# SCLBD/Accelerated-Lpbox-ADMM

Hardware: AMD Instinct MI355X
Metric: admm_iters_per_sec_batched_lp_j100_k500 (higher is better)
Workload: dtype f64

## Files before the change

accelerated-lpbox-admm_amd/csrc/lpbox_dev_common.h:

```cpp
#pragma once
#include <hip/hip_runtime.h>

namespace {

template <int CTRL>
__device__ __forceinline__ double dpp_mov(double v) {
    int lo = __double2loint(v), hi = __double2hiint(v);
    lo = __builtin_amdgcn_mov_dpp(lo, CTRL, 0xf, 0xf, true);
    hi = __builtin_amdgcn_mov_dpp(hi, CTRL, 0xf, 0xf, true);
    return __hiloint2double(hi, lo);
}

struct HalfSwap {
    static __device__ __forceinline__ void run(double a, double b, double &r0, double &r1) {
        auto lo = __builtin_amdgcn_permlane32_swap(__double2loint(a), __double2loint(b), false, false);
        auto hi = __builtin_amdgcn_permlane32_swap(__double2hiint(a), __double2hiint(b), false, false);
        r0 = __hiloint2double(hi[0], lo[0]); r1 = __hiloint2double(hi[1], lo[1]);
    }
};
struct RowSwap {
    static __device__ __forceinline__ void run(double a, double b, double &r0, double &r1) {
        auto lo = __builtin_amdgcn_permlane16_swap(__double2loint(a), __double2loint(b), false, false);
        auto hi = __builtin_amdgcn_permlane16_swap(__double2hiint(a), __double2hiint(b), false, false);
        r0 = __hiloint2double(hi[0], lo[0]); r1 = __hiloint2double(hi[1], lo[1]);
    }
};
template <typename SWAP>
__device__ __forceinline__ double pair_step(double a, double b) { double r0, r1; SWAP::run(a, b, r0, r1); return r0 + r1; }

__device__ __forceinline__ double row_allreduce(double v) {
    v = v + dpp_mov<0xB1>(v);
    v = v + dpp_mov<0x4E>(v);
    v = v + dpp_mov<0x141>(v);
    v = v + dpp_mov<0x140>(v);
    return v;
}

__device__ __forceinline__ double wave_allreduce_sum(double v) {
#ifdef LPBOX_REDUCE_SHFL
    v = v + __shfl_xor(v, 32, 64); v = v + __shfl_xor(v, 16, 64);
    for (int off = 1; off < 16; off <<= 1) v = v + __shfl_xor(v, off, 64);
    return v;
#else
    v = pair_step<HalfSwap>(v, v);
    v = pair_step<RowSwap>(v, v);
    return row_allreduce(v);
#endif
}

template <int NV>
__device__ __forceinline__ double wave_reduce_scatter(const double *v) {
    static_assert(NV >= 2 && NV <= 4, "2..4 values");
    const double x = pair_step<HalfSwap>(v[0], v[1]);
    double s;
    if constexpr (NV == 2) s = pair_step<RowSwap>(x, x);
    else {
        const double y = NV == 4 ? pair_step<HalfSwap>(v[2], v[3]) : pair_step<HalfSwap>(v[2], v[2]);
        s = pair_step<RowSwap>(x, y);
    }
    return row_allreduce(s);
}
__device__ __forceinline__ constexpr int scatter_lane(int nv, int k) { return nv == 2 ? 32 * k : (k == 0 ? 0 : k == 1 ? 32 : k == 2 ? 16 : 48); }

__device__ __forceinline__ int wave_max_int(int v) {
    for (int off = 1; off < 64; off <<= 1) { int o = __shfl_xor(v, off, 64); v = o > v ? o : v; }
    return __builtin_amdgcn_readfirstlane(v);
}

constexpr int RED_MAXV = 6;
constexpr int RED_MAXW = 16;

constexpr int RED_STAGE_BCAST = 0;
constexpr int RED_STAGE_PAIRS = 1;

template <int NV>
__device__ __forceinline__ void wave_partials_store(const double *v, double *buf, int lane, int w) {
    const int row = lane >> 4, k = ((row & 1) << 1) | (row >> 1);
    const bool owner = (lane & 15) == 0;
    double *at = buf + k * RED_MAXW + w;
    if constexpr (NV == 1) {
        const double t0 = wave_allreduce_sum(v[0]);
        if (owner) *at = t0;
    } else {
        constexpr int NS4 = NV > 4 ? 4 : NV;
        const double sc = wave_reduce_scatter<NS4>(v);
        if constexpr (NV == 6) {
            const double sc2 = wave_reduce_scatter<2>(v + 4);
            if (owner) { *at = sc; buf[(4 + (k & 1)) * RED_MAXW + w] = sc2; }
        } else {
            static_assert(NV <= 4, "1, 2, 3, 4 or 6 values");
            if (owner) *at = sc;
        }
    }
}

template <int T, int NV, int STAGE = RED_STAGE_BCAST>
__device__ __forceinline__ void block_sum(double (&v)[NV], double *red, int &parity) {
    constexpr int W = T / 64;
    static_assert(W == 1 || W == 2 || W == 4 || W == 8 || W == 16, "waves per workgroup");
    if constexpr (W == 1) {
#pragma unroll
        for (int k = 0; k < NV; k++) v[k] = wave_allreduce_sum(v[k]);
        return;
    }
    const int lane = threadIdx.x & 63, w = threadIdx.x >> 6;
    double *buf = red + parity * (RED_MAXV * RED_MAXW);
    if constexpr (STAGE != RED_STAGE_BCAST) {
        static_assert(W == 8 && STAGE == RED_STAGE_PAIRS, "built for eight waves");
        wave_partials_store<NV>(v, buf, lane, w);
        __syncthreads();
        double2 t[NV];
#pragma unroll
        for (int k = 0; k < NV; k++) t[k] = *(const double2 *)(buf + k * RED_MAXW + 2 * (lane & 3));
#pragma unroll
        for (int k = 0; k < NV; k++) {
            double u = t[k].x + t[k].y;
            u = u + dpp_mov<0xB1>(u);
            u = u + dpp_mov<0x4E>(u);
            v[k] = u;
        }
        parity ^= 1;
        return;
    }
    if constexpr (NV == 1) {
        const double t0 = wave_allreduce_sum(v[0]);
        if (lane == 0) buf[w] = t0;
    } else {
        constexpr int NS4 = NV > 4 ? 4 : NV;
        const double sc = wave_reduce_scatter<NS4>(v);
#pragma unroll
        for (int k = 0; k < NS4; k++) if (lane == scatter_lane(NS4, k)) buf[k * RED_MAXW + w] = sc;
        if constexpr (NV == 5) {
            const double t4 = wave_allreduce_sum(v[4]);
            if (lane == 0) buf[4 * RED_MAXW + w] = t4;
        } else if constexpr (NV == 6) {
            const double sc2 = wave_reduce_scatter<2>(v + 4);
#pragma unroll
            for (int k = 0; k < 2; k++) if (lane == scatter_lane(2, k)) buf[(4 + k) * RED_MAXW + w] = sc2;
        } else static_assert(NV <= 4, "at most six values");
    }
    __syncthreads();
    if constexpr (W >= 16) {
        double t[NV];
#pragma unroll
        for (int k = 0; k < NV; k++) t[k] = buf[k * RED_MAXW + (lane & (W - 1))];
#pragma unroll
        for (int k = 0; k < NV; k++) v[k] = row_allreduce(t[k]);
        parity ^= 1;
        return;
    }
    double t[NV][W];
#pragma unroll
    for (int k = 0; k < NV; k++)
#pragma unroll
        for (int w2 = 0; w2 < W; w2++) t[k][w2] = buf[k * RED_MAXW + w2];
#pragma unroll
    for (int k = 0; k < NV; k++) {
#pragma unroll
        for (int span = 1; span < W; span <<= 1)
#pragma unroll
            for (int w2 = 0; w2 < W; w2 += 2 * span) t[k][w2] = t[k][w2] + t[k][w2 + span];
        v[k] = t[k][0];
// ... 46 lines not shown
```

accelerated-lpbox-admm_amd/csrc/lpbox_lp_kernels.hip:

```cpp
#include "lpbox_lp.h"
#include "lpbox_dev_common.h"

#include <float.h>

#include <utility>

namespace {

#ifdef LPBOX_STAMPS
#define STAMP_DECL unsigned long long st_acc[16] = {0}; unsigned long long st_t = __builtin_amdgcn_s_memtime();
#define STAMP(k) { __builtin_amdgcn_sched_barrier(0); unsigned long long st_n = __builtin_amdgcn_s_memtime(); \
                   __builtin_amdgcn_s_waitcnt(0xC07F); st_acc[k] += st_n - st_t; st_t = st_n; __builtin_amdgcn_sched_barrier(0); }
#define STAMP_STORE if (tid == 64 * bd.stamp_wave && bd.stamps) { for (int k = 0; k < 16; k++) bd.stamps[(size_t)inst * 16 + k] = st_acc[k]; }
#else
#define STAMP_DECL
#define STAMP(k)
#define STAMP_STORE
#endif
#if defined(LPBOX_STAMPS) && defined(LPBOX_STAMPS_PREBAR)
#define STAMP_PRE(k) STAMP(k)
#define STAMP_POST(k) STAMP(14)
#else
#define STAMP_PRE(k)
#define STAMP_POST(k) STAMP(k)
#endif

#ifndef LPBOX_LP_G1
#define LPBOX_LP_G1 2
#endif
#if !defined(LPBOX_STAMPS) && !defined(LPBOX_KO_COLCAP) && !defined(LPBOX_KO_ROWCAP) && !defined(LPBOX_KO_NOMUL) && !defined(LPBOX_KO_ROWS) && \
    !defined(LPBOX_KO_COLS) && !defined(LPBOX_KO_RED1) && !defined(LPBOX_KO_RED2) && !defined(LPBOX_KO_DIV) && !defined(LPBOX_KO_FIXED_PCG) && LPBOX_LP_G1 == 2
#define LPBOX_PCG_SPEC 1
#else
#define LPBOX_PCG_SPEC 0
#endif
#if LPBOX_PCG_SPEC && !defined(LPBOX_LP_OUTER_LEGACY)
#define LPBOX_OUTER_FUSED 1
#else
#define LPBOX_OUTER_FUSED 0
#endif

struct LdsLayout {
    size_t gx, gl, red, hist, rowf, rowy3, rs_ptr, cs_ptr, hs_ptr, rs_col, cs_row, H, dcol, drow, dmap, total;
    __host__ __device__ LdsLayout(int NS, int LS, int ZS, bool lean, int HL = 0, int HLD = 0) {
        size_t o = 0;
        auto take = [&](size_t bytes) { size_t at = o; o += (bytes + 15) & ~size_t(15); return at; };
        gx = take(sizeof(double) * (2 * (size_t)NS + 3));
        gl = take(sizeof(double) * 3 * ((size_t)LS + 1));
        red = take(sizeof(double) * 2 * RED_MAXV * RED_MAXW);
        hist = take(sizeof(double) * 2 * LP_HIST);
        rowf = take(lean ? sizeof(double) * ((size_t)LS + 1) : 0);
        rowy3 = take(lean ? sizeof(double) * ((size_t)LS + 1) : 0);
        rs_ptr = take(sizeof(int) * ((size_t)NS + 1));
        cs_ptr = take(sizeof(int) * ((size_t)NS + 1));
        hs_ptr = take(sizeof(int) * ((size_t)NS + 1));
        rs_col = take(sizeof(uint16_t) * (size_t)ZS);
        cs_row = take(sizeof(uint16_t) * (size_t)ZS);
        H = take(sizeof(double) * (size_t)HL * (size_t)HLD);
        dcol = take(HL ? sizeof(double) * ((size_t)HL + 1) : 0);
        drow = take(HL ? sizeof(double) * ((size_t)HL + 1) : 0);
        dmap = take(HL ? sizeof(int) * ((size_t)HL + 1) : 0);
        total = o;
    }
};

__host__ __device__ constexpr bool lp_is_lean(int T, int EPT) { return EPT >= 4 || T == 1024; }

__host__ __device__ constexpr int lp_red_stage(int T, int EPT) {
    return T == 512 && EPT == 1 ? RED_STAGE_PAIRS : RED_STAGE_BCAST;
}

constexpr int LP_PCG_RCAP = 12, LP_PCG_CCAP = 12, LP_PCG_HCAP = 8;
__host__ __device__ constexpr bool lp_pcg_scalar_loop(int T, int EPT, bool direct, bool log) { return LPBOX_PCG_SPEC != 0 && T == 512 && EPT == 1 && !direct && !log; }
__host__ __device__ constexpr bool lp_pcg_spec_geometry(int T, int EPT, bool direct, bool log) { return lp_pcg_scalar_loop(T, EPT, direct, log); }
__host__ __device__ constexpr bool lp_pcg_spec_built(int rn, int cn, int hn) {
    return rn >= 0 && rn <= LP_PCG_RCAP / 2 && cn >= 0 && cn <= LP_PCG_CCAP / 2 && hn >= 0 && hn <= LP_PCG_HCAP / 2;
}
__host__ __device__ constexpr bool lp_outer_fused(int T, int EPT, bool direct, bool log) { return LPBOX_OUTER_FUSED != 0 && T == 512 && EPT == 1 && !direct && !log; }

typedef __attribute__((address_space(3))) double lds_double;

__device__ __forceinline__ unsigned lds_addr(const void *p) {
    return (unsigned)(size_t)(__attribute__((address_space(3))) const void *)p;
}
template <int COMP>
__device__ __forceinline__ double lds_ld(unsigned a) {
    return ((const lds_double *)(size_t)a)[COMP];
}

template <int... V>
struct Caps {
    static constexpr int N = sizeof...(V);
    static constexpr int total = (V + ... + 0);
    static constexpr int at(int i) { constexpr int a[N] = {V...}; return a[i]; }
    static constexpr int off(int i) { constexpr int a[N] = {V...}; int o = 0; for (int k = 0; k < i; k++) o += a[k]; return o; }
};

template <typename F, int... I>
__device__ __forceinline__ void static_for_impl(F &&f, std::integer_sequence<int, I...>) {
    (f(std::integral_constant<int, I>{}), ...);
}
template <int N, typename F>
__device__ __forceinline__ void static_for(F &&f) {
    static_for_impl(f, std::make_integer_sequence<int, N>{});
}

template <typename C>
struct Lists {
    unsigned addr[C::total > 0 ? C::total : 1];
    const int *ptr;
    int pos0, pstride;
    int tail_any[C::N];
    static constexpr bool TAILREG = C::N < 4;
    int tail_begin[TAILREG ? C::N : 1], tail_end[TAILREG ? C::N : 1];
    int wlen[C::N];
    unsigned base, zero;
};

template <typename C, int S, int STRIDE>
__device__ __forceinline__ void build_list(Lists<C> &g, int begin, int end, const uint16_t *idx) {
    constexpr int CAP = C::at(S), OFF = C::off(S);
#pragma unroll
    for (int k = 0; k < CAP; k++) g.addr[OFF + k] = (begin + k < end) ? g.base + STRIDE * (unsigned)idx[begin + k] : g.zero;
// ... 268 lines not shown
    }
    __device__ __forceinline__ void load(double *uniform_base, unsigned thread_idx) {
        ub = (char *)uniform_base; boff = thread_idx * 8u;
        if constexpr (MODE != 1) {
#pragma unroll
            for (int s = 0; s < N; s++) r[s] = *elem(s);
        }
    }
    __device__ __forceinline__ double get(int s) const { if constexpr (MODE == 1) return *elem(s); else return r[s]; }
    __device__ __forceinline__ void set(int s, double v) { if constexpr (MODE == 1) *elem(s) = v; else r[s] = v; }
    __device__ __forceinline__ void park(bool dirty = true) {
        if constexpr (MODE == 2) {
            if (dirty) {
#pragma unroll
                for (int s = 0; s < N; s++) *elem(s) = r[s];
            }
        }
    }
    __device__ __forceinline__ void unpark() {
        if constexpr (MODE == 2) {
#pragma unroll
            for (int s = 0; s < N; s++) r[s] = *elem(s);
        }
    }
    __device__ __forceinline__ void store() const {
        if constexpr (MODE != 1) {
#pragma unroll
            for (int s = 0; s < N; s++) *elem(s) = r[s];
        }
    }
};

template <bool MEM, int N, int STRIDE>
struct RowVec {
    double r[MEM ? 1 : N];
    double *lds;
    static __device__ __forceinline__ int at(int idx) {
#ifndef LPBOX_NO_OPAQUE_ROWVEC
        asm volatile("" : "+v"(idx));
#endif
        return idx * STRIDE;
    }
    __device__ __forceinline__ double get(int s, int idx, bool leader) const {
        if constexpr (MEM) return leader ? lds[at(idx)] : 0.0; else return r[s];
    }
    __device__ __forceinline__ void set(int s, int idx, bool leader, double v) {
        if constexpr (MEM) { if (leader) lds[at(idx)] = v; } else r[s] = v;
    }
};

template <int T, int EPT, typename RCAPS, typename CCAPS, typename HCAPS, bool DIRECT = false, bool LOG = false>
__global__ void __launch_bounds__(T) lp_window_kernel(LpBatchDev bd, int iter_start, int iter_end, int mode) {
    const int l2f = mode & 1, rec = mode & 2;
    constexpr int RS = (DIRECT || LOG) ? RED_STAGE_BCAST : lp_red_stage(T, EPT);
    constexpr bool SCALAR_LOOP = lp_pcg_scalar_loop(T, EPT, DIRECT, LOG), SPEC = lp_pcg_spec_geometry(T, EPT, DIRECT, LOG);
    constexpr bool FUSED = lp_outer_fused(T, EPT, DIRECT, LOG);
    auto uni = [](bool c) { if constexpr (SCALAR_LOOP) return __builtin_amdgcn_ballot_w64(c) != 0; else return c; };
    extern __shared__ __attribute__((aligned(16))) unsigned char smem[];
    const int inst = blockIdx.x, tid = threadIdx.x;
    int *isc = bd.isc + (size_t)inst * NI_COUNT;
    double *dsc = bd.dsc + (size_t)inst * ND_COUNT;
    if (!isc[NI_ACTIVE]) return;

    const int nnz = isc[NI_NNZ];
    const size_t on = (size_t)inst * bd.NS, ol = (size_t)inst * bd.LS, oz = (size_t)inst * bd.ZS;

    static_assert(!DIRECT || EPT == 1, "the direct x-update is built for the one-slot variants");
    const LdsLayout L(bd.NS, bd.LS, bd.ZS, lp_is_lean(T, EPT), DIRECT ? bd.HL : 0, DIRECT ? bd.HLD : 0);
    double *gx = (double *)(smem + L.gx);
    double *gl = (double *)(smem + L.gl);
    double *red = (double *)(smem + L.red);
    double *s_hist = (double *)(smem + L.hist);
    int *s_rs_ptr = (int *)(smem + L.rs_ptr);
    int *s_cs_ptr = (int *)(smem + L.cs_ptr);
    int *s_hs_ptr = (int *)(smem + L.hs_ptr);
    uint16_t *s_rs_col = (uint16_t *)(smem + L.rs_col);
    uint16_t *s_cs_row = (uint16_t *)(smem + L.cs_row);

    {
        const int *gp = bd.rs_ptr + (size_t)inst * (bd.NS + 1);
        const int *gc = bd.cs_ptr + (size_t)inst * (bd.NS + 1);
        const int *gh = bd.hs_ptr + (size_t)inst * (bd.NS + 1);
        for (int i = tid; i <= bd.NS; i += T) { s_rs_ptr[i] = gp[i]; s_cs_ptr[i] = gc[i]; s_hs_ptr[i] = gh[i]; }
        const uint16_t *c0 = bd.rs_col + oz, *r0 = bd.cs_row + oz;
        for (int k = tid; k < nnz; k += T) { s_rs_col[k] = c0[k]; s_cs_row[k] = r0[k]; }
        if (tid == 0) { gx[bd.NS] = 0.0; gx[2 * bd.NS + 2] = 0.0; gl[3 * bd.LS] = 0.0; gl[3 * bd.LS + 1] = 0.0; gl[3 * bd.LS + 2] = 0.0; }
    }
    double *Hm = (double *)(smem + L.H), *dcol = (double *)(smem + L.dcol), *drow = (double *)(smem + L.drow);
    int *dmap = (int *)(smem + L.dmap);
    int h_valid = 0;
    if constexpr (DIRECT) {
        h_valid = isc[NI_H_VALID];
        const size_t hsz = (size_t)bd.HL * bd.HLD;
        if (h_valid) { const double *Hg = bd.H + (size_t)inst * (hsz + bd.LS); for (size_t e = tid; e < hsz; e += T) Hm[e] = Hg[e]; }
    }

    constexpr bool LEAN = lp_is_lean(T, EPT);
    double x[EPT], dinv[EPT];
    SlotVec<LEAN ? 2 : 0, EPT, T> z1, z2, b;
    SlotVec<LEAN ? 1 : 0, EPT, T> pd;
    z1.load(bd.z1 + on, (unsigned)tid); z2.load(bd.z2 + on, (unsigned)tid); b.load(bd.b + on, (unsigned)tid); pd.load(bd.pd + on, (unsigned)tid);
    double Esq_reg[LEAN ? 1 : EPT];
    if constexpr (!LEAN) {
#pragma unroll
        for (int s = 0; s < EPT; s++) Esq_reg[s] = (double)(bd.cmeta[on + s * T + tid] & 0x7FFF);
    }
    auto Esq = [&](int s) { if constexpr (LEAN) return (double)(bd.cmeta[on + s * T + tid] & 0x7FFF); else return Esq_reg[s]; };
    bool live[EPT];
    double Ex[EPT];
    RowVec<LEAN, EPT, 3> z4;
    RowVec<LEAN, EPT, 1> f, y3;
    z4.lds = gl + 1; f.lds = (double *)(smem + L.rowf); y3.lds = (double *)(smem + L.rowy3);
    int rinfo[EPT], rGreg[LEAN ? 1 : EPT];
    bool rvreg[LEAN ? 1 : EPT];
    auto rgl = [&](int s) { return rinfo[s] & 0xFFFF; };
    auto rG = [&](int s) { if constexpr (LEAN) return (rinfo[s] >> 16) & 15; else return rGreg[s]; };
    auto rvalid = [&](int s) { if constexpr (LEAN) return (rinfo[s] & (1 << 20)) != 0; else return rvreg[s]; };
#pragma unroll
    for (int s = 0; s < EPT; s++) {
        const int pos = s * T + tid;
        x[s] = bd.x[on + pos];
        live[s] = bd.live[on + pos] != 0;
        const int rid = bd.rid[on + pos], meta = bd.rmeta[on + pos];
        const bool rtask = rid != 0xFFFF, leader = rtask && (meta & 15) == 0;
        rinfo[s] = rtask ? ((int)bd.rgl[on + pos] | ((meta >> 4) << 16) | (leader ? 1 << 20 : 0)) : (1 << 16);
        if constexpr (!LEAN) { rinfo[s] &= 0xFFFF; rGreg[s] = rtask ? (meta >> 4) : 1; rvreg[s] = leader; }
        z4.set(s, rgl(s), leader, leader ? bd.z4[ol + rid] : 0.0);
        f.set(s, rgl(s), leader, leader ? bd.f[ol + rid] : 0.0);
        y3.set(s, rgl(s), leader, 0.0);
        Ex[s] = 0.0;
    }
    int gdir = -1;
    double wrow = 0.0;
    if constexpr (DIRECT) {
        if (rvalid(0)) {
            gdir = bd.rdir[on + tid];
            if (gdir >= 0) dmap[gdir] = rgl(0);
            if (h_valid) wrow = bd.H[(size_t)inst * ((size_t)bd.HL * bd.HLD + bd.LS) + (size_t)bd.HL * bd.HLD + rgl(0)];
            gl[3 * rgl(0) + 2] = 0.0;
        }
    }
    double rho1 = dsc[ND_RHO1], rho2 = dsc[ND_RHO2], rho4 = dsc[ND_RHO4];
    double prev_rho1 = dsc[ND_PREV_RHO1], prev_rho2 = dsc[ND_PREV_RHO2], prev_rho4 = dsc[ND_PREV_RHO4];
    double gamma_val = dsc[ND_GAMMA], dI = dsc[ND_DI], r4Et = dsc[ND_R4ET], rcr = dsc[ND_RCR];
    double std_obj = dsc[ND_STD_OBJ], cur_obj = dsc[ND_CUR_OBJ], best_bin_obj = dsc[ND_BEST_BIN_OBJ];
    double sum_fix_obj = dsc[ND_SUM_FIX_OBJ], fix_obj = dsc[ND_FIX_OBJ], c1 = dsc[ND_C1];
    double cvg1 = dsc[ND_CVG1], cvg2 = dsc[ND_CVG2], obj_val = dsc[ND_OBJ_VAL];
    double prev_sum = dsc[ND_PREV_SUM], prev_obj = dsc[ND_PREV_OBJ];
    int n_live = isc[NI_NLIVE], rhoUpdated = isc[NI_RHO_UPDATED], hist_n = isc[NI_HIST_N];
    int pcg_total = isc[NI_PCG_TOTAL], outer_total = isc[NI_OUTER_TOTAL], last_pcg = isc[NI_LAST_PCG];
    int expr_ready = isc[NI_EXPR_READY];
    int hbuf = 0;
    double h_reg[LEAN ? 1 : LP_HIST];
    if constexpr (LEAN) { if (tid < LP_HIST) s_hist[tid] = bd.hist[(size_t)inst * LP_HIST + tid]; }
    else {
#pragma unroll
        for (int k = 0; k < LP_HIST; k++) h_reg[k] = bd.hist[(size_t)inst * LP_HIST + k];
    }
    const double learning_fact = LP_LEARNING_FACT;
    int ret = 0, stop = LP_STOP_NONE, parity = 0;

    __syncthreads();

    static_assert(RCAPS::N == EPT && CCAPS::N == EPT && HCAPS::N == EPT, "one capacity per slot");
    Lists<RCAPS> rl;
    Lists<CCAPS> cl;
    Lists<HCAPS> hl;
    bool clong[EPT];
    int anyhelp[EPT];
    rl.base = lds_addr(gx); rl.zero = lds_addr(gx + bd.NS);
    rl.ptr = s_rs_ptr; cl.ptr = s_cs_ptr; hl.ptr = s_hs_ptr;
    rl.pos0 = cl.pos0 = hl.pos0 = tid; rl.pstride = cl.pstride = hl.pstride = T;
    cl.base = lds_addr(gl); cl.zero = lds_addr(gl + 3 * bd.LS);
    hl.base = cl.base; hl.zero = cl.zero;
    int rGmax[EPT];
    static_for<EPT>([&](auto S) {
        constexpr int s = decltype(S)::value;
        const int pos = s * T + tid;
        build_list<RCAPS, s, 8>(rl, s_rs_ptr[pos], s_rs_ptr[pos + 1], s_rs_col);
        rGmax[s] = wave_max_int(rG(s));
        build_list<CCAPS, s, 24>(cl, s_cs_ptr[pos], s_cs_ptr[pos + 1], s_cs_row);
        build_list<HCAPS, s, 24>(hl, s_hs_ptr[pos], s_hs_ptr[pos + 1], s_cs_row);
        const int cm = bd.cmeta[on + pos];
        clong[s] = (cm & 0x8000) != 0;
        anyhelp[s] = wave_max_int(s_hs_ptr[pos + 1] - s_hs_ptr[pos]) > 0;
    });
    int spec_rn = 0, spec_cn = 0, spec_hn = 0;
    bool spec_ok = false;
    if constexpr (SPEC) {
        static_assert(RCAPS::at(0) == LP_PCG_RCAP && CCAPS::at(0) == LP_PCG_CCAP && HCAPS::at(0) == LP_PCG_HCAP, "capacities of the 512 x 1 kernel");
        spec_rn = (rl.wlen[0] + 1) / 2; spec_cn = (cl.wlen[0] + 1) / 2; spec_hn = (hl.wlen[0] + 1) / 2;
        spec_ok = !bd.pcg_generic && !(rl.tail_any[0] | cl.tail_any[0] | hl.tail_any[0]);
    }
    auto op_add = [](double acc, double v) { return acc + v; };
    constexpr int GX2 = T * EPT + 2;
    auto rows_combine = [&](const double (&part)[EPT], double (&out)[EPT]) {
        static_for<EPT>([&](auto S) {
            constexpr int s = decltype(S)::value;
            double v = part[s];
            if (rGmax[s] >= 2) { const double u = v + dpp_mov<0xB1>(v); v = rG(s) >= 2 ? u : v; }
            if (rGmax[s] >= 4) { const double u = v + dpp_mov<0x4E>(v); v = rG(s) >= 4 ? u : v; }
            if (rGmax[s] >= 8) { const double u = v + dpp_mov<0x141>(v); v = rG(s) >= 8 ? u : v; }
            out[s] = v;
        });
    };
    auto rows_gather_at = [&](auto COMPC, double (&out)[EPT]) {
        double part[EPT];
        if constexpr (LEAN) touch_list(rl);
        gather_all<RCAPS, 8, decltype(COMPC)::value>(rl, s_rs_col, op_add, part);
        rows_combine(part, out);
    };
    auto rows_gather = [&](double (&out)[EPT]) { rows_gather_at(std::integral_constant<int, 0>{}, out); };

// ... 290 lines not shown
                            const int j = tid & 127;
                            if (j < nG) {
                                const double rk = drow[j];
                                for (int i = tid >> 7; i < nG; i += T / 128) {
                                    const double ck = dcol[i];
                                    const double cur = Hm[i * HLD + j];
                                    Hm[i * HLD + j] = i == k ? rk : (j == k ? -(ck * piv) : cur - ck * rk);
                                }
                            }
                        }
                        __syncthreads();
                    }
                    {
                        double *Hg = bd.H + (size_t)inst * ((size_t)bd.HL * HLD + bd.LS);
                        for (int e = tid; e < bd.HL * HLD; e += T) Hg[e] = Hm[e];
                        if (rvalid(0)) Hg[(size_t)bd.HL * HLD + rgl(0)] = wrow;
                    }
                    h_valid = 1;
                }
                const double q1 = apply_Q(rhs[0]);
                gx[tid] = live[0] ? q1 : 0.0;
                __syncthreads();
                {
                    double t[EPT];
                    rows_gather(t);
                    if (rvalid(0) && gdir >= 0) dcol[gdir] = t[0];
                }
                __syncthreads();
                for (int i = tid >> 2; i < nG; i += T / 4) {
                    const double *Hr = Hm + i * HLD;
                    double acc = 0.0;
#pragma unroll 4
                    for (int j = tid & 3; j < nG; j += 4) acc = acc + Hr[j] * dcol[j];
                    const double u = quad_sum(acc);
                    if ((tid & 3) == 0) gl[3 * dmap[i] + 2] = u;
                }
                __syncthreads();
                double v[EPT];
                cols_gather(std::integral_constant<int, 2>{}, op_add, v);
                const double yv = rhs[0] - v[0];
                xt[0] = apply_Q(yv) / dI;
            } else {
            double r[EPT], p[EPT];
            double p3[3] = {0.0, 0.0, 0.0};
            double tcol[EPT];
            if constexpr (FUSED) tcol[0] = tcf[0];
            else
            cols_gather(std::integral_constant<int, 2>{}, op_add, tcol);
#pragma unroll
            for (int s = 0; s < EPT; s++) {
                const double t = tcol[s];
                xt[s] = y1[s];
                double Mx = 0.0;
                Mx += dI * (1.0 * xt[s]);
                Mx += t;
                r[s] = rhs[s] - Mx;
                p[s] = dinv[s] * r[s];
                p3[0] = p3[0] + (live[s] ? rhs[s] * rhs[s] : 0.0);
                p3[1] = p3[1] + (live[s] ? r[s] * r[s] : 0.0);
                p3[2] = p3[2] + (live[s] ? r[s] * p[s] : 0.0);
            }
            block_sum<T, 3, RS>(p3, red, parity);
            STAMP(2)
            const double rhsNorm2 = p3[0];
            double residualNorm2 = p3[1], absNew = p3[2];
            if (uni(rhsNorm2 == 0)) {
#pragma unroll
                for (int s = 0; s < EPT; s++) xt[s] = 0.0;
            } else {
                double threshold = LP_PCG_TOL * LP_PCG_TOL * rhsNorm2;
                if (threshold < DBL_MIN) threshold = DBL_MIN;
                if constexpr (SCALAR_LOOP) {
                    auto pcg_loop = [&](auto RKC, auto CKC, auto HKC) {
                        constexpr int RK = decltype(RKC)::value, CK = decltype(CKC)::value, HK = decltype(HKC)::value;
                        static_assert((RK >= 0) == (CK >= 0) && (RK >= 0) == (HK >= 0) && (RK < 0 || EPT == 1), "all three lists or none");
                        while (k_it < LP_PCG_MAXITERS) {
#pragma unroll
                            for (int s = 0; s < EPT; s++) gx[s * T + tid] = live[s] ? p[s] : 0.0;
                            __syncthreads();
                            {
                                double q[EPT];
                                if constexpr (RK >= 0) {
                                    double v[RK > 0 ? RK * LPBOX_LP_G1 : 1], part[EPT];
                                    list_read<0, RK>(rl, v);
                                    part[0] = list_sum<RK>(v, op_add);
                                    rows_combine(part, q);
                                } else rows_gather(q);
#pragma unroll
                                for (int s = 0; s < EPT; s++) if (rvalid(s)) gl[3 * rgl(s)] = r4 * q[s];
                            }
                            __syncthreads();
                            double tmp[EPT];
                            double p1[1] = {0.0};
                            if constexpr (CK >= 0) {
                                double vo[CK > 0 ? CK * LPBOX_LP_G1 : 1], vh[HK > 0 ? HK * LPBOX_LP_G1 : 1];
                                list_read<0, CK>(cl, vo);
                                const double own = list_sum<CK>(vo, op_add);
                                __builtin_amdgcn_sched_barrier(0);
                                list_read<0, HK>(hl, vh);
                                if constexpr (HK > 0) {
                                    const double ht = quad_sum(list_sum<HK>(vh, op_add));
                                    tcol[0] = clong[0] ? own + ht : own;
                                } else tcol[0] = own;
                            } else cols_gather(std::integral_constant<int, 0>{}, op_add, tcol);
#pragma unroll
                            for (int s = 0; s < EPT; s++) {
                                const double t = tcol[s];
                                double Mp = 0.0;
                                Mp += dI * (1.0 * p[s]);
                                Mp += t;
                                tmp[s] = Mp;
                                p1[0] = p1[0] + (live[s] ? p[s] * tmp[s] : 0.0);
                            }
                            block_sum<T, 1, RS>(p1, red, parity);
                            const double alpha = absNew / p1[0];
                            if (uni(alpha < 0)) { pcg_fail = true; break; }
                            double p2[2] = {0.0, 0.0};
                            double z[EPT];
#pragma unroll
                            for (int s = 0; s < EPT; s++) {
                                xt[s] += alpha * p[s];
                                r[s] -= alpha * tmp[s];
                                z[s] = dinv[s] * r[s];
                                p2[0] = p2[0] + (live[s] ? r[s] * r[s] : 0.0);
                                p2[1] = p2[1] + (live[s] ? r[s] * z[s] : 0.0);
                            }
                            block_sum<T, 2, RS>(p2, red, parity);
                            residualNorm2 = p2[0];
                            if (uni(residualNorm2 < threshold)) { k_it++; break; }
                            const double absOld = absNew;
                            absNew = p2[1];
                            const double beta = absNew / absOld;
#pragma unroll
                            for (int s = 0; s < EPT; s++) p[s] = z[s] + beta * p[s];
                            k_it++;
                        }
                    };
                    constexpr std::integral_constant<int, -1> GEN{};
                    if (uni(!(residualNorm2 < threshold))) {
                        if constexpr (SPEC) {
                            bool ran = false;
                            if (spec_ok) {
                                dispatch_chunks<LP_PCG_RCAP / 2>(spec_rn, [&](auto R) {
                                    dispatch_chunks<LP_PCG_CCAP / 2>(spec_cn, [&](auto Cn) {
                                        dispatch_chunks<LP_PCG_HCAP / 2>(spec_hn, [&](auto H) {
                                            if constexpr (lp_pcg_spec_built(decltype(R)::value, decltype(Cn)::value, decltype(H)::value)) {
                                                pcg_loop(R, Cn, H);
                                                ran = true;
                                            }
                                        });
                                    });
                                });
                            }
                            if (!ran) pcg_loop(GEN, GEN, GEN);
                        } else pcg_loop(GEN, GEN, GEN);
                    }
                } else {
                if (!(residualNorm2 < threshold)) {
                    while (k_it < LP_PCG_MAXITERS) {
#pragma unroll
                        for (int s = 0; s < EPT; s++) gx[s * T + tid] = live[s] ? p[s] : 0.0;
                        STAMP_PRE(12)
                        __syncthreads();
                        STAMP(3)
                        {
                            double q[EPT];
#ifdef LPBOX_KO_ROWS
                            for (int s = 0; s < EPT; s++) q[s] = p[s];
#else
                            rows_gather(q);
#endif
                            STAMP(4)
#pragma unroll
#ifdef LPBOX_KO_NOMUL
                            for (int s = 0; s < EPT; s++) if (rvalid(s)) gl[3 * rgl(s)] = q[s];
#else
                            for (int s = 0; s < EPT; s++) if (rvalid(s)) gl[3 * rgl(s)] = r4 * q[s];
#endif
// ... 95 lines not shown
                z1.set(s, z1.get(s) + g1 * (x[s] - y1[s]));
                z2.set(s, z2.get(s) + g2 * (x[s] - y2[s]));
                gx[s * T + tid] = live[s] ? x[s] : 0.0;
            }
            if constexpr (FUSED) {
                const bool step = (it + 1) % LP_RHO_STEP == 0;
                start_vec(step ? learning_fact * rho1 : rho1);
                r4n = step ? learning_fact * r4Et : r4Et;
            }
            __syncthreads();
            if constexpr (FUSED) rows_gather_x_y1(Ex, qn);
            else
            rows_gather(Ex);
#pragma unroll
            for (int s = 0; s < EPT; s++) {
                if constexpr (LEAN) {
                    if (rvalid(s)) {
                        const int i = RowVec<true, EPT, 1>::at(rgl(s));
                        const double d = g4 * ((Ex[s] + y3.lds[i]) - f.lds[i]);
                        const double z4o = z4.lds[3 * i];
                        z4.lds[3 * i] = (!l2f && it == iter_start) ? d : z4o + d;
                    }
                } else {
                const double d = g4 * ((Ex[s] + y3.get(s, rgl(s), rvalid(s))) - f.get(s, rgl(s), rvalid(s)));
                z4.set(s, rgl(s), rvalid(s), (!l2f && it == iter_start) ? d : z4.get(s, rgl(s), rvalid(s)) + d);
                }
            }
            double lg[6] = {0.0, 0.0, 0.0, 0.0, 0.0, 0.0};
            if constexpr (LOG) {
#pragma unroll
                for (int s = 0; s < EPT; s++) {
                    const double vy3 = y3.get(s, rgl(s), rvalid(s)), vz4 = z4.get(s, rgl(s), rvalid(s));
                    lg[0] = lg[0] + (live[s] ? y1[s] * y1[s] : 0.0);
                    lg[1] = lg[1] + (live[s] ? y2[s] * y2[s] : 0.0);
                    lg[2] = lg[2] + (rvalid(s) ? vy3 * vy3 : 0.0);
                    lg[3] = lg[3] + (live[s] ? z1.get(s) * z1.get(s) : 0.0);
                    lg[4] = lg[4] + (live[s] ? z2.get(s) * z2.get(s) : 0.0);
                    lg[5] = lg[5] + (rvalid(s) ? vz4 * vz4 : 0.0);
                }
            }
            const bool rho_step = (it + 1) % LP_RHO_STEP == 0;
            double p5[6] = {0.0, 0.0, 0.0, 0.0, 0.0, 0.0};
            p5[5] = prepare(rho_step ? learning_fact * rho1 : rho1, rho_step ? learning_fact * rho2 : rho2, rho_step ? learning_fact * rho4 : rho4);
#pragma unroll
            for (int s = 0; s < EPT; s++) {
                const double d1 = x[s] - y1[s], d2 = x[s] - y2[s];
                const double xb = x[s] >= 0.5 ? 1.0 : 0.0;
                p5[0] = p5[0] + (live[s] ? x[s] * x[s] : 0.0);
                p5[1] = p5[1] + (live[s] ? d1 * d1 : 0.0);
                p5[2] = p5[2] + (live[s] ? d2 * d2 : 0.0);
                p5[3] = p5[3] + (live[s] ? b.get(s) * x[s] : 0.0);
                p5[4] = p5[4] + (live[s] ? b.get(s) * xb : 0.0);
            }
            STAMP_POST(12)
            block_sum<T, 6, RS>(p5, red, parity);
            if constexpr (LOG) block_sum<T, 6, RS>(lg, red, parity);
            pnorm = p5[5];
            STAMP_POST(13)
            {
                const double xn = sqrt(p5[0]);
                const double temp0 = (xn < 2.2204e-16) ? 2.2204e-16 : xn;
                cvg1 = sqrt(p5[1]) / temp0;
                cvg2 = sqrt(p5[2]) / temp0;
            }
            if (cvg1 <= LP_STOP_THRESHOLD && cvg2 <= LP_STOP_THRESHOLD && (l2f || it != iter_start)) {
                if (l2f) ret = 1;
                stop = LP_STOP_Y1Y2;
                break;
            }
            if (rho_step) {
                prev_rho1 = rho1; prev_rho2 = rho2;
                rho1 = learning_fact * rho1;
                rho2 = learning_fact * rho2;
                prev_rho4 = rho4;
                rho4 = learning_fact * rho4;
                const double g = gamma_val * LP_GAMMA_FACTOR;
                gamma_val = g < 1.0 ? 1.0 : g;
                rhoUpdated = 1;
                rcr = learning_fact - 1.0;
            }
            obj_val = p5[3];
            double h[LP_HIST];
            if constexpr (LEAN) {
                const double *hs = s_hist + hbuf * LP_HIST;
#pragma unroll
                for (int k = 0; k < LP_HIST; k++) h[k] = hs[k];
            } else {
#pragma unroll
                for (int k = 0; k < LP_HIST; k++) h[k] = h_reg[k];
            }
            if (hist_n < LP_HIST) {
#pragma unroll
                for (int k = 0; k < LP_HIST; k++) if (k == hist_n) h[k] = obj_val;
            } else {
#pragma unroll
                for (int k = 0; k < LP_HIST - 1; k++) h[k] = h[k + 1];
                h[LP_HIST - 1] = obj_val;
            }
            if constexpr (LEAN) {
                hbuf ^= 1;
                if (tid == 0) {
#pragma unroll
                    for (int k = 0; k < LP_HIST; k++) s_hist[hbuf * LP_HIST + k] = h[k];
                }
            } else {
#pragma unroll
                for (int k = 0; k < LP_HIST; k++) h_reg[k] = h[k];
            }
            if (hist_n < 0x3fffffff) hist_n++;
            if (hist_n >= LP_HIST) {
                double mean = 0;
#pragma unroll
                for (int k = 0; k < LP_HIST; k++) mean += h[k];
                mean /= (double)LP_HIST;
                double dev = 0;
#pragma unroll
                for (int k = 0; k < LP_HIST; k++) dev += (h[k] - mean) * (h[k] - mean);
                dev /= (double)(LP_HIST - 1);
                const double sd = (dev == 0) ? 0.0 : sqrt(dev);
                std_obj = sd / fabs(h[LP_HIST - 1]);
            }
            if (std_obj <= LP_STD_THRESHOLD) { ret = 1; stop = LP_STOP_OBJSTD; break; }
            cur_obj = p5[4];
            if (best_bin_obj >= cur_obj) best_bin_obj = cur_obj;
            if constexpr (LOG) {
                if (tid == 0 && bd.logbuf && it - iter_start < bd.log_cap) {
                    double *lr = bd.logbuf + ((size_t)inst * bd.log_cap + (it - iter_start)) * LP_LOG_VALS;
                    lr[0] = (double)k_it; lr[1] = sqrt(p5[0]);
#pragma unroll
                    for (int k = 0; k < 6; k++) lr[2 + k] = sqrt(lg[k]);
                    lr[8] = obj_val; lr[9] = cur_obj; lr[10] = (double)(wall_clock64() - log_t0); lr[11] = (double)it;
                }
            }
            if constexpr (LEAN) {
                rho1 = uniform_f64(rho1); rho2 = uniform_f64(rho2); rho4 = uniform_f64(rho4);
                prev_rho1 = uniform_f64(prev_rho1); prev_rho2 = uniform_f64(prev_rho2); prev_rho4 = uniform_f64(prev_rho4);
                gamma_val = uniform_f64(gamma_val); rcr = uniform_f64(rcr); dI = uniform_f64(dI); r4Et = uniform_f64(r4Et);
                std_obj = uniform_f64(std_obj); cur_obj = uniform_f64(cur_obj); best_bin_obj = uniform_f64(best_bin_obj);
                cvg1 = uniform_f64(cvg1); cvg2 = uniform_f64(cvg2); obj_val = uniform_f64(obj_val); pnorm = uniform_f64(pnorm);
            }
            STAMP(14)
        }
        STAMP_STORE
    }

    z1.store(); z2.store(); pd.store();
#pragma unroll
    for (int s = 0; s < EPT; s++) {
        const int pos = s * T + tid;
        {
            bd.x[on + pos] = x[s];
            bd.live[on + pos] = live[s] ? 1 : 0;
        }
        if (rvalid(s)) { const int rid = bd.rid[on + pos]; bd.z4[ol + rid] = z4.get(s, rgl(s), true); bd.f[ol + rid] = f.get(s, rgl(s), true); }
    }
    if (tid == 0) {
        dsc[ND_RHO1] = rho1; dsc[ND_RHO2] = rho2; dsc[ND_RHO4] = rho4;
        dsc[ND_PREV_RHO1] = prev_rho1; dsc[ND_PREV_RHO2] = prev_rho2; dsc[ND_PREV_RHO4] = prev_rho4;
        dsc[ND_GAMMA] = gamma_val; dsc[ND_DI] = dI; dsc[ND_R4ET] = r4Et; dsc[ND_RCR] = rcr;
        dsc[ND_STD_OBJ] = std_obj; dsc[ND_CUR_OBJ] = cur_obj; dsc[ND_BEST_BIN_OBJ] = best_bin_obj;
        dsc[ND_SUM_FIX_OBJ] = sum_fix_obj; dsc[ND_FIX_OBJ] = fix_obj; dsc[ND_C1] = c1;
        dsc[ND_CVG1] = cvg1; dsc[ND_CVG2] = cvg2; dsc[ND_OBJ_VAL] = obj_val;
        dsc[ND_PREV_SUM] = prev_sum; dsc[ND_PREV_OBJ] = prev_obj;
        isc[NI_NLIVE] = n_live; isc[NI_RHO_UPDATED] = rhoUpdated; isc[NI_HIST_N] = hist_n;
        isc[NI_RET] = ret; isc[NI_STOP] = stop;
        isc[NI_PCG_TOTAL] = pcg_total; isc[NI_OUTER_TOTAL] = outer_total; isc[NI_LAST_PCG] = last_pcg;
        isc[NI_EXPR_READY] = expr_ready;
        if constexpr (DIRECT) isc[NI_H_VALID] = h_valid;
        if (l2f) isc[NI_ITER] = it;
        else isc[NI_PLAIN_ITER_P1] = it + 1;
        for (int k = 0; k < LP_HIST; k++) bd.hist[(size_t)inst * LP_HIST + k] = LEAN ? s_hist[hbuf * LP_HIST + k] : h_reg[LEAN ? 0 : k];
    }
}

__global__ void lp_pack_xiters_kernel(LpBatchDev bd, const int *live_pos, const int *rows, int ws, double *out,
                                      long out_stride) {
    const int inst = blockIdx.y;
    const int nr = rows[inst];
    const long total = (long)nr * ws;
    const double *xh = bd.xhist + (size_t)inst * bd.ws_cap * bd.NS;
    const int *li = live_pos + (size_t)inst * bd.NS;
    double *o = out + (size_t)inst * out_stride;
    for (long e = (long)blockIdx.x * blockDim.x + threadIdx.x; e < total; e += (long)gridDim.x * blockDim.x) {
        const int r = (int)(e / ws), c = (int)(e % ws);
        o[e] = xh[(size_t)c * bd.NS + li[r]];
    }
}

template <int T, int NV, int STAGE>
__global__ void __launch_bounds__(T) debug_block_sum_kernel(const double *in, double *out, int rounds) {
    __shared__ __attribute__((aligned(16))) double red[2 * RED_MAXV * RED_MAXW];
    const int tid = threadIdx.x;
    int parity = 0;
    for (int r = 0; r < rounds; r++) {
        double v[NV];
#pragma unroll
        for (int k = 0; k < NV; k++) v[k] = in[((size_t)r * T + tid) * NV + k];
        block_sum<T, NV, STAGE>(v, red, parity);
#pragma unroll
        for (int k = 0; k < NV; k++) out[(((size_t)blockIdx.x * rounds + r) * T + tid) * NV + k] = v[k];
    }
}

}

hipError_t lp_launch_debug_block_sum(int T, int NV, int stage, int groups, int rounds, const double *in, double *out, hipStream_t s) {
#define CALL_DBG(TT, VV, SS)                                                                                             \
    if (T == TT && NV == VV && stage == SS) {                                                                           \
        hipLaunchKernelGGL((debug_block_sum_kernel<TT, VV, SS>), dim3(groups), dim3(TT), 0, s, in, out, rounds);      \
        return hipGetLastError();                                                                                     \
    }
#define CALL_DBG_NV(TT, SS) CALL_DBG(TT, 1, SS) CALL_DBG(TT, 2, SS) CALL_DBG(TT, 3, SS) CALL_DBG(TT, 6, SS)
    CALL_DBG_NV(256, RED_STAGE_BCAST) CALL_DBG_NV(512, RED_STAGE_BCAST) CALL_DBG_NV(1024, RED_STAGE_BCAST)
    CALL_DBG_NV(512, RED_STAGE_PAIRS)
#undef CALL_DBG_NV
#undef CALL_DBG
    return hipErrorInvalidConfiguration;
}

size_t lp_window_lds_bytes(int T, int NS, int LS, int ZS, int HL, int HLD) {
    return LdsLayout(NS, LS, ZS, lp_is_lean(T, NS / T), HL, HLD).total;
}

bool lp_pcg_specialised(int T, int EPT) { return lp_pcg_spec_geometry(T, EPT, false, false); }
void lp_pcg_list_caps(int *rows, int *cols, int *help) { *rows = LP_PCG_RCAP; *cols = LP_PCG_CCAP; *help = LP_PCG_HCAP; }
bool lp_direct_supported(int T, int EPT) { return T == 512 && EPT == 1; }
bool lp_log_supported(int T, int EPT) { return T == 512 && (EPT == 1 || EPT == 2 || EPT == 4); }

#define LP_DISPATCH(KERNEL_CALL)                                                                                                          \
    if (T == 256 && EPT == 1) { KERNEL_CALL(256, 1, (Caps<12>), (Caps<12>), (Caps<8>)) }                                                     \
    else if (T == 256 && EPT == 2) { KERNEL_CALL(256, 2, (Caps<12, 12>), (Caps<12, 8>), (Caps<8, 4>)) }                                       \
    else if (T == 256 && EPT == 4) { KERNEL_CALL(256, 4, (Caps<12, 12, 12, 12>), (Caps<24, 8, 8, 8>), (Caps<0, 0, 0, 0>)) }                  \
    else if (T == 256 && EPT == 8) { KERNEL_CALL(256, 8, (Caps<8, 8, 8, 8, 8, 8, 8, 8>), (Caps<8, 8, 8, 8, 4, 4, 4, 4>), (Caps<0, 0, 0, 0, 0, 0, 0, 0>)) } \
    else if (T == 512 && EPT == 1) { KERNEL_CALL(512, 1, (Caps<12>), (Caps<12>), (Caps<8>)) }                                                \
    else if (T == 512 && EPT == 2) { KERNEL_CALL(512, 2, (Caps<12, 12>), (Caps<12, 8>), (Caps<8, 4>)) }                                      \
    else if (T == 512 && EPT == 4) { KERNEL_CALL(512, 4, (Caps<12, 8, 8, 8>), (Caps<12, 8, 8, 8>), (Caps<8, 4, 4, 4>)) }                        \
    else if (T == 1024 && EPT == 1) { KERNEL_CALL(1024, 1, (Caps<8>), (Caps<8>), (Caps<8>)) }                                                \
    else if (T == 1024 && EPT == 2) { KERNEL_CALL(1024, 2, (Caps<8, 8>), (Caps<8, 8>), (Caps<4, 4>)) }                                     \
    else return hipErrorInvalidConfiguration;

#define LP_UNPAREN(...) __VA_ARGS__

hipError_t lp_launch_init(const LpBatchDev &bd, int T, int EPT, const double *f_org, const double *c1_init,
                          const uint8_t *live_init, hipStream_t s) {
#define CALL_INIT(TT, EE, RR, CCC, HHH) hipLaunchKernelGGL((lp_init_kernel<TT, EE>), dim3(bd.B), dim3(TT), 0, s, bd, f_org, c1_init, live_init);
    LP_DISPATCH(CALL_INIT)
#undef CALL_INIT
    return hipGetLastError();
}

hipError_t lp_launch_window(const LpBatchDev &bd, int T, int EPT, size_t lds, int iter_start, int iter_end, int l2f,
                            hipStream_t s, bool direct, bool log) {
    if (log) {
        if (direct || !lp_log_supported(T, EPT) || bd.logbuf == nullptr) return hipErrorInvalidConfiguration;
#define CALL_LOG(EE, RR, CCC, HHH)                                                                             \
    {                                                                                                          \
        auto kfn = lp_window_kernel<512, EE, LP_UNPAREN RR, LP_UNPAREN CCC, LP_UNPAREN HHH, false, true>;      \
        hipError_t e = hipFuncSetAttribute((const void *)kfn, hipFuncAttributeMaxDynamicSharedMemorySize, (int)lds); \
        if (e != hipSuccess) return e;                                                                         \
        hipLaunchKernelGGL(kfn, dim3(bd.B), dim3(512), lds, s, bd, iter_start, iter_end, l2f);                 \
    }
        if (EPT == 1) CALL_LOG(1, (Caps<12>), (Caps<12>), (Caps<8>))
        else if (EPT == 2) CALL_LOG(2, (Caps<12, 12>), (Caps<12, 8>), (Caps<8, 4>))
        else CALL_LOG(4, (Caps<12, 8, 8, 8>), (Caps<12, 8, 8, 8>), (Caps<8, 4, 4, 4>))
#undef CALL_LOG
        return hipGetLastError();
    }
// ... 32 lines not shown
```

Measured before the change: 8.068 million.

## Add lazy stop tests, dead-lane zeroing, low-half reductions and mean prefix in LP kernel

Several independent micro-optimizations are added to the 512-thread, EPT=1 fused LP window kernel. Convergence and objective-std tests compare squared quantities against the squared threshold with a safety margin, deferring the sqrt/div work and computing exact values only at exit. Dead lanes are zeroed once so the PCG loop can drop per-element live predicates. Wave reductions feed undefined values into the unused swap half to save moves. The history mean is partially precomputed before the block reduction. Together these trim ALU and latency on the critical per-iteration path, at the cost of more code-path complexity and reliance on the margin-based inequality being conservative.

```diff
diff --git a/accelerated-lpbox-admm_amd/csrc/lpbox_dev_common.h b/accelerated-lpbox-admm_amd/csrc/lpbox_dev_common.h
--- a/accelerated-lpbox-admm_amd/csrc/lpbox_dev_common.h
+++ b/accelerated-lpbox-admm_amd/csrc/lpbox_dev_common.h
@@ -27,6 +27,15 @@
 };
 template <typename SWAP>
 __device__ __forceinline__ double pair_step(double a, double b) { double r0, r1; SWAP::run(a, b, r0, r1); return r0 + r1; }
+
+__device__ __forceinline__ double undefined_f64() {
+    int lo, hi;
+    asm volatile("" : "=v"(lo));
+    asm volatile("" : "=v"(hi));
+    return __hiloint2double(hi, lo);
+}
+template <typename SWAP>
+__device__ __forceinline__ double pair_step_low(double a) { double r0, r1; SWAP::run(a, undefined_f64(), r0, r1); return r0 + r1; }
 
 __device__ __forceinline__ double row_allreduce(double v) {
     v = v + dpp_mov<0xB1>(v);
@@ -72,15 +81,27 @@
 
 constexpr int RED_STAGE_BCAST = 0;
 constexpr int RED_STAGE_PAIRS = 1;
-
-template <int NV>
+constexpr int RED_STAGE_PAIRS_LOW = 2;
+
+template <int NV, bool LOW = false>
 __device__ __forceinline__ void wave_partials_store(const double *v, double *buf, int lane, int w) {
     const int row = lane >> 4, k = ((row & 1) << 1) | (row >> 1);
     const bool owner = (lane & 15) == 0;
     double *at = buf + k * RED_MAXW + w;
     if constexpr (NV == 1) {
-        const double t0 = wave_allreduce_sum(v[0]);
+        double t0;
+        if constexpr (LOW) t0 = row_allreduce(pair_step_low<RowSwap>(pair_step_low<HalfSwap>(v[0])));
+        else t0 = wave_allreduce_sum(v[0]);
         if (owner) *at = t0;
+    } else if constexpr (LOW && NV == 2) {
+        const double x = pair_step<HalfSwap>(v[0], v[1]);
+        const double sc = row_allreduce(pair_step_low<RowSwap>(x));
+        if (owner) *at = sc;
+    } else if constexpr (LOW && NV == 3) {
+        const double x = pair_step<HalfSwap>(v[0], v[1]);
+        const double y = pair_step_low<HalfSwap>(v[2]);
+        const double sc = row_allreduce(pair_step<RowSwap>(x, y));
+        if (owner) *at = sc;
     } else {
         constexpr int NS4 = NV > 4 ? 4 : NV;
         const double sc = wave_reduce_scatter<NS4>(v);
@@ -106,8 +127,8 @@
     const int lane = threadIdx.x & 63, w = threadIdx.x >> 6;
     double *buf = red + parity * (RED_MAXV * RED_MAXW);
     if constexpr (STAGE != RED_STAGE_BCAST) {
-        static_assert(W == 8 && STAGE == RED_STAGE_PAIRS, "built for eight waves");
-        wave_partials_store<NV>(v, buf, lane, w);
+        static_assert(W == 8 && (STAGE == RED_STAGE_PAIRS || STAGE == RED_STAGE_PAIRS_LOW), "built for eight waves");
+        wave_partials_store<NV, STAGE == RED_STAGE_PAIRS_LOW>(v, buf, lane, w);
         __syncthreads();
         double2 t[NV];
 #pragma unroll
diff --git a/accelerated-lpbox-admm_amd/csrc/lpbox_lp_kernels.hip b/accelerated-lpbox-admm_amd/csrc/lpbox_lp_kernels.hip
--- a/accelerated-lpbox-admm_amd/csrc/lpbox_lp_kernels.hip
+++ b/accelerated-lpbox-admm_amd/csrc/lpbox_lp_kernels.hip
@@ -1,5 +1,6 @@
 #include "lpbox_lp.h"
 #include "lpbox_dev_common.h"
+#include "lpbox_lp_stoptest.h"
 
 #include <float.h>
 
@@ -38,6 +39,21 @@
 #define LPBOX_OUTER_FUSED 1
 #else
 #define LPBOX_OUTER_FUSED 0
+#endif
+#ifndef LPBOX_LP_LAZYSTOP
+#define LPBOX_LP_LAZYSTOP 1
+#endif
+#ifndef LPBOX_LP_MEANPREFIX
+#define LPBOX_LP_MEANPREFIX 1
+#endif
+#ifndef LPBOX_LP_DEADZERO
+#define LPBOX_LP_DEADZERO 1
+#endif
+#ifndef LPBOX_LP_REDLOW
+#define LPBOX_LP_REDLOW 1
+#endif
+#ifndef LPBOX_LP_MPDIRECT
+#define LPBOX_LP_MPDIRECT 1
 #endif
 
 struct LdsLayout {
@@ -69,6 +85,9 @@
 __host__ __device__ constexpr int lp_red_stage(int T, int EPT) {
     return T == 512 && EPT == 1 ? RED_STAGE_PAIRS : RED_STAGE_BCAST;
 }
+__host__ __device__ constexpr bool lp_lean_stream(int T, int EPT, bool direct, bool log, int step_on) {
+    return LPBOX_OUTER_FUSED != 0 && step_on != 0 && T == 512 && EPT == 1 && !direct && !log;
+}
 
 constexpr int LP_PCG_RCAP = 12, LP_PCG_CCAP = 12, LP_PCG_HCAP = 8;
 __host__ __device__ constexpr bool lp_pcg_scalar_loop(int T, int EPT, bool direct, bool log) { return LPBOX_PCG_SPEC != 0 && T == 512 && EPT == 1 && !direct && !log; }
@@ -443,7 +462,10 @@
 template <int T, int EPT, typename RCAPS, typename CCAPS, typename HCAPS, bool DIRECT = false, bool LOG = false>
 __global__ void __launch_bounds__(T) lp_window_kernel(LpBatchDev bd, int iter_start, int iter_end, int mode) {
     const int l2f = mode & 1, rec = mode & 2;
-    constexpr int RS = (DIRECT || LOG) ? RED_STAGE_BCAST : lp_red_stage(T, EPT);
+    constexpr bool LAZY = lp_lean_stream(T, EPT, DIRECT, LOG, LPBOX_LP_LAZYSTOP), DEADZ = lp_lean_stream(T, EPT, DIRECT, LOG, LPBOX_LP_DEADZERO);
+    constexpr bool MPDIR = lp_lean_stream(T, EPT, DIRECT, LOG, LPBOX_LP_MPDIRECT), MEANPRE = lp_lean_stream(T, EPT, DIRECT, LOG, LPBOX_LP_MEANPREFIX);
+    constexpr int RS = (DIRECT || LOG) ? RED_STAGE_BCAST
+                     : lp_lean_stream(T, EPT, DIRECT, LOG, LPBOX_LP_REDLOW) ? RED_STAGE_PAIRS_LOW : lp_red_stage(T, EPT);
     constexpr bool SCALAR_LOOP = lp_pcg_scalar_loop(T, EPT, DIRECT, LOG), SPEC = lp_pcg_spec_geometry(T, EPT, DIRECT, LOG);
     constexpr bool FUSED = lp_outer_fused(T, EPT, DIRECT, LOG);
     auto uni = [](bool c) { if constexpr (SCALAR_LOOP) return __builtin_amdgcn_ballot_w64(c) != 0; else return c; };
@@ -550,6 +572,8 @@
     }
     const double learning_fact = LP_LEARNING_FACT;
     int ret = 0, stop = LP_STOP_NONE, parity = 0;
+    bool cvg_pending = false, std_pending = false;
+    double pend_a1 = 0.0, pend_a2 = 0.0, pend_c = 0.0, pend_devq = 0.0, pend_h9 = 0.0;
 
     __syncthreads();
 
@@ -946,6 +970,8 @@
                 const double t = tcol[s];
                 xt[s] = y1[s];
                 double Mx = 0.0;
+                if constexpr (MPDIR) Mx = dI * (1.0 * xt[s]);
+                else
                 Mx += dI * (1.0 * xt[s]);
                 Mx += t;
                 r[s] = rhs[s] - Mx;
@@ -954,6 +980,8 @@
                 p3[1] = p3[1] + (live[s] ? r[s] * r[s] : 0.0);
                 p3[2] = p3[2] + (live[s] ? r[s] * p[s] : 0.0);
             }
+            double dz[1] = {0.0};
+            if constexpr (DEADZ) { r[0] = live[0] ? r[0] : 0.0; p[0] = live[0] ? p[0] : 0.0; dz[0] = live[0] ? dinv[0] : 0.0; }
             block_sum<T, 3, RS>(p3, red, parity);
             STAMP(2)
             const double rhsNorm2 = p3[0];
@@ -970,7 +998,7 @@
                         static_assert((RK >= 0) == (CK >= 0) && (RK >= 0) == (HK >= 0) && (RK < 0 || EPT == 1), "all three lists or none");
                         while (k_it < LP_PCG_MAXITERS) {
 #pragma unroll
-                            for (int s = 0; s < EPT; s++) gx[s * T + tid] = live[s] ? p[s] : 0.0;
+                            for (int s = 0; s < EPT; s++) gx[s * T + tid] = (DEADZ || live[s]) ? p[s] : 0.0;
                             __syncthreads();
                             {
                                 double q[EPT];
@@ -1001,10 +1029,12 @@
                             for (int s = 0; s < EPT; s++) {
                                 const double t = tcol[s];
                                 double Mp = 0.0;
+                                if constexpr (MPDIR) Mp = dI * (1.0 * p[s]);
+                                else
                                 Mp += dI * (1.0 * p[s]);
                                 Mp += t;
                                 tmp[s] = Mp;
-                                p1[0] = p1[0] + (live[s] ? p[s] * tmp[s] : 0.0);
+                                p1[0] = p1[0] + ((DEADZ || live[s]) ? p[s] * tmp[s] : 0.0);
                             }
                             block_sum<T, 1, RS>(p1, red, parity);
                             const double alpha = absNew / p1[0];
@@ -1015,9 +1045,9 @@
                             for (int s = 0; s < EPT; s++) {
                                 xt[s] += alpha * p[s];
                                 r[s] -= alpha * tmp[s];
-                                z[s] = dinv[s] * r[s];
+                                z[s] = (DEADZ ? dz[0] : dinv[s]) * r[s];
                                 p2[0] = p2[0] + (live[s] ? r[s] * r[s] : 0.0);
-                                p2[1] = p2[1] + (live[s] ? r[s] * z[s] : 0.0);
+                                p2[1] = p2[1] + ((DEADZ || live[s]) ? r[s] * z[s] : 0.0);
                             }
                             block_sum<T, 2, RS>(p2, red, parity);
                             residualNorm2 = p2[0];
@@ -1219,18 +1249,32 @@
                 p5[3] = p5[3] + (live[s] ? b.get(s) * x[s] : 0.0);
                 p5[4] = p5[4] + (live[s] ? b.get(s) * xb : 0.0);
             }
+            bool hist_full = false;
+            double mean_pre = 0.0;
+            if constexpr (MEANPRE) {
+                hist_full = hist_n >= LP_HIST;
+                if (hist_full) {
+#pragma unroll
+                    for (int k = 1; k < LP_HIST; k++) mean_pre += h_reg[LEAN ? 0 : k];
+                }
+            }
             STAMP_POST(12)
             block_sum<T, 6, RS>(p5, red, parity);
             if constexpr (LOG) block_sum<T, 6, RS>(lg, red, parity);
             pnorm = p5[5];
             STAMP_POST(13)
+            if constexpr (LAZY) {
+                cvg_pending = uni(lp_cvg_certainly_above(p5[1], p5[0], LP_STOP_THRESHOLD) || lp_cvg_certainly_above(p5[2], p5[0], LP_STOP_THRESHOLD));
+                pend_a1 = p5[1]; pend_a2 = p5[2]; pend_c = p5[0];
+            }
+            if (!cvg_pending)
             {
                 const double xn = sqrt(p5[0]);
                 const double temp0 = (xn < 2.2204e-16) ? 2.2204e-16 : xn;
                 cvg1 = sqrt(p5[1]) / temp0;
                 cvg2 = sqrt(p5[2]) / temp0;
             }
-            if (cvg1 <= LP_STOP_THRESHOLD && cvg2 <= LP_STOP_THRESHOLD && (l2f || it != iter_start)) {
+            if (!cvg_pending && cvg1 <= LP_STOP_THRESHOLD && cvg2 <= LP_STOP_THRESHOLD && (l2f || it != iter_start)) {
                 if (l2f) ret = 1;
                 stop = LP_STOP_Y1Y2;
                 break;
@@ -1277,17 +1321,32 @@
             if (hist_n < 0x3fffffff) hist_n++;
             if (hist_n >= LP_HIST) {
                 double mean = 0;
+                if constexpr (MEANPRE) {
+                    if (hist_full) mean = mean_pre + h[LP_HIST - 1];
+                    else {
+#pragma unroll
+                        for (int k = 0; k < LP_HIST; k++) mean += h[k];
+                    }
+                } else {
 #pragma unroll
                 for (int k = 0; k < LP_HIST; k++) mean += h[k];
+                }
                 mean /= (double)LP_HIST;
                 double dev = 0;
 #pragma unroll
                 for (int k = 0; k < LP_HIST; k++) dev += (h[k] - mean) * (h[k] - mean);
                 dev /= (double)(LP_HIST - 1);
+                if constexpr (LAZY) {
+                    std_pending = uni(lp_std_certainly_above(dev, h[LP_HIST - 1], LP_STD_THRESHOLD));
+                    pend_devq = dev; pend_h9 = h[LP_HIST - 1];
+                }
+                if (!std_pending)
+                {
                 const double sd = (dev == 0) ? 0.0 : sqrt(dev);
                 std_obj = sd / fabs(h[LP_HIST - 1]);
-            }
-            if (std_obj <= LP_STD_THRESHOLD) { ret = 1; stop = LP_STOP_OBJSTD; break; }
+                }
+            }
+            if (!std_pending && std_obj <= LP_STD_THRESHOLD) { ret = 1; stop = LP_STOP_OBJSTD; break; }
             cur_obj = p5[4];
             if (best_bin_obj >= cur_obj) best_bin_obj = cur_obj;
             if constexpr (LOG) {
@@ -1311,6 +1370,10 @@
         STAMP_STORE
     }
 
+    if constexpr (LAZY) {
+        if (cvg_pending) { cvg1 = lp_cvg_exact(pend_a1, pend_c); cvg2 = lp_cvg_exact(pend_a2, pend_c); }
+        if (std_pending) std_obj = lp_std_exact(pend_devq, pend_h9);
+    }
     z1.store(); z2.store(); pd.store();
 #pragma unroll
     for (int s = 0; s < EPT; s++) {
@@ -1379,7 +1442,7 @@
     }
 #define CALL_DBG_NV(TT, SS) CALL_DBG(TT, 1, SS) CALL_DBG(TT, 2, SS) CALL_DBG(TT, 3, SS) CALL_DBG(TT, 6, SS)
     CALL_DBG_NV(256, RED_STAGE_BCAST) CALL_DBG_NV(512, RED_STAGE_BCAST) CALL_DBG_NV(1024, RED_STAGE_BCAST)
-    CALL_DBG_NV(512, RED_STAGE_PAIRS)
+    CALL_DBG_NV(512, RED_STAGE_PAIRS) CALL_DBG_NV(512, RED_STAGE_PAIRS_LOW)
 #undef CALL_DBG_NV
 #undef CALL_DBG
     return hipErrorInvalidConfiguration;
diff --git a/accelerated-lpbox-admm_amd/csrc/lpbox_lp_stoptest.h b/accelerated-lpbox-admm_amd/csrc/lpbox_lp_stoptest.h
--- /dev/null
+++ b/accelerated-lpbox-admm_amd/csrc/lpbox_lp_stoptest.h
@@ -0,0 +1,30 @@
+#pragma once
+#include <math.h>
+
+#if defined(__HIPCC__) || defined(__CUDACC__)
+#define LPBOX_STOP_HD __host__ __device__ __forceinline__
+#else
+#define LPBOX_STOP_HD inline
+#endif
+
+#define LPBOX_STOP_MARGIN (1.0 + 0x1p-30)
+
+LPBOX_STOP_HD double lp_cvg_exact(double a, double c) {
+    const double xn = sqrt(c);
+    const double temp0 = (xn < 2.2204e-16) ? 2.2204e-16 : xn;
+    return sqrt(a) / temp0;
+}
+LPBOX_STOP_HD bool lp_cvg_certainly_above(double a, double c, double T) {
+    const double inf = __builtin_huge_val();
+    return a < inf && c < inf && c >= 0x1p-100 && a > ((T * T) * c) * LPBOX_STOP_MARGIN;
+}
+
+LPBOX_STOP_HD double lp_std_exact(double devq, double h9) {
+    const double sd = (devq == 0) ? 0.0 : sqrt(devq);
+    return sd / fabs(h9);
+}
+LPBOX_STOP_HD bool lp_std_certainly_above(double devq, double h9, double S) {
+    const double inf = __builtin_huge_val();
+    const double ah = fabs(h9), sh = S * ah;
+    return devq < inf && ah >= 0x1p-400 && ah <= 0x1p400 && devq > (sh * sh) * LPBOX_STOP_MARGIN;
+}
```

Result: faster. 8.396 million (median of 6 runs) (+4.1%).
